# zzbuzzard/PATHS

Hardware: AMD Instinct MI355X
Metric: slides_per_sec_5level_K2048_D1024 (higher is better)
Workload: dtype f32 (products as 2 fp16 planes per operand = 22 bits, 3 fp16 MFMAs per block, fp32 accumulate); 1 GPU; 5-level PATHS recursion (forward, eval): K=2048 patches/level (level-0 grid 32x64, top_k 512, 10% background), D=1024 features, trans_dim 128 x 4 heads x 2 layers, LSTM ctx 256; 8 HBM-resident slides per GPU; slides_per_gpu=8, global_batch=8, levels=5, resident_batches_rotated=3, parallelism=slide-sharded x1 (no data-path collective)

## Files before the change

paths_amd/csrc/gemm_epi.h:

```cpp
#pragma once
#include "common.h"

namespace paths_epi {



struct TileView {
  char* base; int64_t ldb; uint32_t lane_off;
  __device__ TileView(const float* p, int64_t ld, int lane)
      : base(reinterpret_cast<char*>(const_cast<float*>(p))), ldb(ld * 4), lane_off((uint32_t)((4 * (lane >> 5)) * ld + (lane & 31)) * 4u) {}
  __device__ float* at(int trow, int tcol, int r) const {
    char* tile = base + (int64_t)trow * ldb + (int64_t)tcol * 4;
    const uint32_t off = lane_off + (uint32_t)((r & 3) + 8 * (r >> 2)) * (uint32_t)ldb;
    return reinterpret_cast<float*>(tile + off);
  }
  __device__ char* tile(int trow, int tcol) const { return base + (int64_t)trow * ldb + (int64_t)tcol * 4; }
  __device__ float* elem(char* tile_origin, int r) const {
    return reinterpret_cast<float*>(tile_origin + (lane_off + (uint32_t)((r & 3) + 8 * (r >> 2)) * (uint32_t)ldb));
  }
  __device__ float* at_clamped(int trow, int tcol, int r, int lane, int M) const {
    const int row = min(trow + c32_row(r, lane), M - 1);
    return reinterpret_cast<float*>(base + (int64_t)row * ldb + (int64_t)(tcol + (lane & 31)) * 4);
  }
};
// ... 220 lines not shown
      char* to = ovw.tile(trow, tcol); char* tx = xvw.tile(trow, tcol);
      if constexpr (RAW_O) {
        const f32x4* t4 = reinterpret_cast<const f32x4*>(o + ((int64_t)(trow >> 5) * (N >> 5) + (tcol >> 5)) * 1024) + lane;
#pragma unroll
        for (int q = 0; q < 4; ++q) {
          const f32x4 v = t4[64 * q];
          ov[s][4 * q] = v[0]; ov[s][4 * q + 1] = v[1]; ov[s][4 * q + 2] = v[2]; ov[s][4 * q + 3] = v[3];
        }
      }
      static_for<0, 16>([&](auto rc) __attribute__((always_inline)) {
        constexpr int r = decltype(rc)::value;
        if constexpr (FULL) {
          if constexpr (!RAW_O) ov[s][r] = *ovw.elem(to, r);
          if constexpr (WITH_Y) xv[s][r] = *xvw.elem(tx, r);
        } else {
          if constexpr (!RAW_O) ov[s][r] = *ovw.at_clamped(trow, tcol, r, lane, M);
          if constexpr (WITH_Y) xv[s][r] = *xvw.at_clamped(trow, tcol, r, lane, M);
        }
      });
    };
    static_for<0, (PD < NT ? PD : NT)>([&](auto tc) __attribute__((always_inline)) { load(tc); });
    static_for<0, NT>([&](auto tc) __attribute__((always_inline)) {
      constexpr int t = decltype(tc)::value, i = t % WTM, j = t / WTM, s = t % NB;
      if constexpr (t + PD < NT) load(std::integral_constant<int, t + PD>{});
      const int trow = row0 + 32 * i, tcol = col0 + 32 * j;
      if (tcol < N) {
        const float b = bias[tcol + (lane & 31)];
        char* th = hv.tile(trow, tcol); char* ty = yv.tile(trow, tcol); char* tt = tv.tile(trow, tcol);
        static_for<0, 16>([&](auto rc) __attribute__((always_inline)) {
          constexpr int r = decltype(rc)::value;
          const float tcv = tanh_acc(fmaf(acc[i][j][r], acc_scale, b));
          const float h = (RAW_O ? sigmoid_acc(ov[s][r]) : ov[s][r]) * tcv;
          if constexpr (FULL) {
            if constexpr (WITH_TC) *tv.elem(tt, r) = tcv;
            *hv.elem(th, r) = h;
            if constexpr (WITH_Y) *yv.elem(ty, r) = xv[s][r] + h;
          } else if (tile_row_ok<false>(trow, r, lane, M)) {
            if constexpr (WITH_TC) *tv.at_clamped(trow, tcol, r, lane, M) = tcv;
            *hv.at_clamped(trow, tcol, r, lane, M) = h;
            if constexpr (WITH_Y) *yv.at_clamped(trow, tcol, r, lane, M) = xv[s][r] + h;
          }
        });
      }
      __builtin_amdgcn_sched_barrier(0);
    });
  }
  template <int WTM, int WTN, int WGM, int WGN>
  __device__ __forceinline__ void run(f32x16 (&acc)[WTM][WTN], int row0, int col0, int lane, int, int, int M, float*) const {
    if (row0 + 32 * WTM <= M) run_impl<true>(acc, row0, col0, lane, M);
    else run_impl<false>(acc, row0, col0, lane, M);
  }
};

struct EpiBias {
  template <int WTM, int WTN>
  __device__ __forceinline__ void init(f32x16 (&acc)[WTM][WTN], int, int, int, int) const {
#pragma unroll
    for (int i = 0; i < WTM; ++i)
#pragma unroll
      for (int j = 0; j < WTN; ++j)
#pragma unroll
        for (int r = 0; r < 16; ++r) acc[i][j][r] = 0.f;
  }

  const float* bias; float* out; int64_t ldo; int N; int act;
  const float* residual; int64_t ldr; const float* mask; int64_t ldm; int accumulate;
  float acc_scale = 1.0f;
  template <bool FULL, int WTM, int WTN>
  __device__ __forceinline__ void run_impl(f32x16 (&acc)[WTM][WTN], int row0, int col0, int lane, int M) const {
    constexpr int NT = WTM * WTN;
    const TileView outv(out, ldo, lane), resv(residual, ldr, lane), maskv(mask, ldm, lane);
    float rv[2][16], mv[2][16], ov[2][16];
    const bool any_load = residual != nullptr || mask != nullptr || accumulate != 0;
    auto load = [&](auto tc) __attribute__((always_inline)) {
      constexpr int t = decltype(tc)::value, i = t % WTM, j = t / WTM, s = t & 1;
      const int trow = row0 + 32 * i, tcol = col0 + 32 * j;
      const int lcol = min(tcol + (lane & 31), N - 1) - (lane & 31);
#pragma unroll
      for (int r = 0; r < 16; ++r) {
        rv[s][r] = residual ? *tile_elem<FULL>(resv, trow, lcol, r, lane, M) : 0.f;
        mv[s][r] = mask ? *tile_elem<FULL>(maskv, trow, lcol, r, lane, M) : 1.f;
        ov[s][r] = accumulate ? *tile_elem<FULL>(outv, trow, lcol, r, lane, M) : 0.f;
      }
    };
    if (any_load) load(std::integral_constant<int, 0>{});
    static_for<0, NT>([&](auto tc) __attribute__((always_inline)) {
      constexpr int t = decltype(tc)::value, i = t % WTM, j = t / WTM, s = t & 1;
      if constexpr (t + 1 < NT) {
        if (any_load) load(std::integral_constant<int, t + 1>{});
      }
      const int trow = row0 + 32 * i, tcol = col0 + 32 * j;
      const int colr = tcol + (lane & 31);
      const float b = bias ? bias[min(colr, N - 1)] : 0.f;
      if (tcol < N) {
#pragma unroll
        for (int r = 0; r < 16; ++r) {
          float v = fmaf(acc[i][j][r], acc_scale, b);
          if (act == 1) v = fmaxf(v, 0.f);
          if (any_load) {
            if (!(mv[s][r] > 0.f)) v = 0.f;
            v += rv[s][r] + ov[s][r];
          }
          if (tile_row_ok<FULL>(trow, r, lane, M) && (tcol + 32 <= N || colr < N)) *tile_elem<FULL>(outv, trow, tcol, r, lane, M) = v;
        }
      }
      __builtin_amdgcn_sched_barrier(0);
// ... 188 lines not shown
```

paths_amd/csrc/gemm_x6.hip:

```cpp
#include "common.h"
#include "gemm_epi.h"
#include "finish_qkv.h"

#ifndef PATHS_X6_PART
#define PATHS_X6_PART 0
#endif

namespace {
using namespace paths_epi;

typedef __bf16 bf16x8 __attribute__((ext_vector_type(8)));
typedef _Float16 f16x8 __attribute__((ext_vector_type(8)));
typedef _Float16 f16x2 __attribute__((ext_vector_type(2)));
typedef __bf16 bf16x2 __attribute__((ext_vector_type(2)));
typedef float f32x2 __attribute__((ext_vector_type(2)));
typedef uint32_t u32x2 __attribute__((ext_vector_type(2)));
typedef uint32_t u32x4 __attribute__((ext_vector_type(4)));

__device__ __forceinline__ uint32_t pk_bf16(float a, float b) {
  f32x2 v = {a, b};
  return __builtin_bit_cast(uint32_t, __builtin_convertvector(v, bf16x2));
}
__device__ __forceinline__ float bf_lo(uint32_t p) { return __builtin_bit_cast(float, p << 16); }
__device__ __forceinline__ float bf_hi(uint32_t p) { return __builtin_bit_cast(float, p & 0xffff0000u); }

__device__ __forceinline__ uint32_t pk_f16(float a, float b) {
  f32x2 v = {a, b};
  return __builtin_bit_cast(uint32_t, __builtin_convertvector(v, f16x2));
}
__device__ __forceinline__ float h_lo(uint32_t p) { return (float)__builtin_bit_cast(f16x2, p)[0]; }
__device__ __forceinline__ float h_hi(uint32_t p) { return (float)__builtin_bit_cast(f16x2, p)[1]; }

constexpr int FRAG = 1024;
template <int NP> constexpr int planes_of() { return NP == 4 ? 2 : NP; }
template <int NP> constexpr int subt() { return planes_of<NP>() * FRAG; }

struct X6Operands {
  const float* A0; int64_t lda0; int K0;
  const int64_t* A0rows;
  const float* A1; int64_t lda1; int K1;
  const float* Aadd; int64_t ldadd;
  const char* Wt;
  int64_t w_group_stride;
  int M;
  const int64_t* num_ims;
  int rows_per_slide;
  float a_scale;
  int ksplit = 1;
};

template <int NP, int WTM, int WTN, int PF, bool ADD, bool ROWS, class Epi, int OCC = 1, bool A16 = false>
__global__ void __launch_bounds__(256) __attribute__((amdgpu_waves_per_eu(OCC, OCC)))
gemm_x6_kernel(X6Operands g, Epi epi) {
  static_assert(NP == 2 || NP == 3 || NP == 4, "two fp16 planes, three bf16 planes or two bf16 planes");
  static_assert(!A16 || (NP == 2 && ROWS), "fp16 A rows: two-plane fp16 split, row-pointer form");
  constexpr int PL = planes_of<NP>();
  constexpr bool A1P = A16 && !ADD;
  constexpr int PLA = A1P ? 1 : PL;
  constexpr int SUBT = subt<NP>();
  constexpr int SUBTA = PLA * FRAG;
  constexpr int NPROD = NP == 3 ? 6 : A1P ? 2 : 3;
  constexpr int BM = WTM * 64, BN = WTN * 64;
  constexpr int SA = 2 * WTM, SB = 2 * WTN;
  constexpr int STAGE = SA * SUBTA + SB * SUBT;
  constexpr int NA = BM / 64;
  constexpr int NPB = SB * PL, NB = (NPB + 3) / 4;
  static_assert(WTM % 2 == 0, "A fragment register slots alternate per accumulator row");
  extern __shared__ __attribute__((aligned(16))) char smem[];
  const int tid = threadIdx.x, lane = tid & 63, wave = __builtin_amdgcn_readfirstlane(tid >> 6), wm = wave >> 1, wn = wave & 1;

  const int nbx = gridDim.x, nby = gridDim.y, nblk = nbx * nby;
  int lin = blockIdx.y * nbx + blockIdx.x;
  {
    const int q = nblk >> 3, r = nblk & 7, xcd = lin & 7, j = lin >> 3;
    lin = (xcd < r ? xcd * (q + 1) : r * (q + 1) + (xcd - r) * q) + j;
  }
  constexpr int GM = 8;
  const int per_group = GM * nbx;
  const int grp = lin / per_group, in_grp = lin - grp * per_group;
  const int rows_in_grp = min(GM, nby - grp * GM);
  const int by = grp * GM + in_grp % rows_in_grp, bx = in_grp / rows_in_grp;
  const int m0 = by * BM, n0 = bx * BN;
  if (block_all_padding(g.num_ims, g.rows_per_slide, m0, BM, g.M)) return;

  const int arow = tid >> 2, ac = tid & 3;
  uint32_t aoff0[NA], aoff1[NA], aoffs[ADD ? NA : 1]; int awr[NA];
  typedef const f32x4 __attribute__((address_space(1))) * gptr_f4;
  typedef const u32x2 __attribute__((address_space(1))) * gptr_h4;
  gptr_f4 rowp[ROWS && !A16 ? NA : 1];
  gptr_h4 rowh[A16 ? NA : 1];
#pragma unroll
  for (int p = 0; p < NA; ++p) {
    const int row = p * 64 + arow;
    const int64_t grow = min(m0 + row, g.M - 1);
    aoff0[p] = ROWS ? 0u : (uint32_t)((grow * g.lda0 + 4 * ac) * 4);
    if constexpr (A16) rowh[p] = reinterpret_cast<gptr_h4>(static_cast<uintptr_t>(g.A0rows[grow]) + 8 * ac);
    else if constexpr (ROWS) rowp[p] = reinterpret_cast<gptr_f4>(static_cast<uintptr_t>(g.A0rows[grow]) + 16 * ac);
    aoff1[p] = (uint32_t)((grow * g.lda1 + 4 * ac) * 4);
    if constexpr (ADD) aoffs[p] = (uint32_t)((grow * g.ldadd + 4 * ac) * 4);
    awr[p] = (row >> 5) * SUBTA + (ac >> 1) * 512 + (row & 31) * 16 + (ac & 1) * 8;
  }
  const int K0w = g.ksplit > 1 ? g.K0 / g.ksplit : g.K0;
  const int kofs = g.ksplit > 1 ? (int)blockIdx.z * K0w : 0;
  if (kofs != 0) {
#pragma unroll
    for (int p = 0; p < NA; ++p) {
      aoff0[p] += (uint32_t)kofs * 4u;
      if constexpr (A16) rowh[p] += kofs >> 2;
      else if constexpr (ROWS) rowp[p] += kofs >> 2;
      if constexpr (ADD) aoffs[p] += (uint32_t)kofs * 4u;
    }
  }
  const int nk0 = K0w >> 4, nk = (K0w + g.K1) >> 4;
  const char* bbase[NB]; int bwr[NB];
#pragma unroll
  for (int i = 0; i < NB; ++i) {
    int pc = wave + 4 * i;
    if (pc >= NPB) pc -= 4;
    const int sub = pc / PL, pl = pc % PL;
    bbase[i] = g.Wt + ((int64_t)(n0 >> 5) + sub) * g.w_group_stride + pl * FRAG;
    bwr[i] = (A1P ? SA * SUBTA + sub * SUBT : (SA + sub) * SUBT) + pl * FRAG + lane * 16;
  }
  static_assert(PF == 1 || PF == 2, "one or two register sets");
  f32x4 sa[PF][NA], sadd[ADD ? PF : 1][ADD ? NA : 1]; u32x4 sbr[PF][NB];
  u32x2 sh[A16 ? PF : 1][A16 ? NA : 1];
  uint32_t hi[NA][2], mid[NP != 2 ? NA : 1][2], lo[NA][2];
  float* const anyA = const_cast<float*>(ROWS ? reinterpret_cast<const float*>(g.Wt) : g.A0);
  const auto rsA0 = __builtin_amdgcn_make_buffer_rsrc(anyA, 0, 0xFFFFFFFFu, 0x00020000);
  const auto rsA1 = __builtin_amdgcn_make_buffer_rsrc(g.A1 ? const_cast<float*>(g.A1) : anyA, 0, 0xFFFFFFFFu, 0x00020000);
  const auto rsAdd = __builtin_amdgcn_make_buffer_rsrc(ADD ? const_cast<float*>(g.Aadd) : anyA, 0, 0xFFFFFFFFu, 0x00020000);
  const auto rsW = __builtin_amdgcn_make_buffer_rsrc(const_cast<char*>(g.Wt), 0, 0xFFFFFFFFu, 0x00020000);
  const int lane16 = lane * 16;
  int bsoff[NB];
#pragma unroll
  for (int i = 0; i < NB; ++i) bsoff[i] = (int)(bbase[i] - g.Wt) + (kofs >> 4) * SUBT;
  auto gload_a = [&](int set, int q, int kt) {
// ... 34 lines not shown
        asm("v_pk_mul_f16 %0, %1, %2" : "=v"(hi[q][1]) : "v"(sh[set][q][1]), "v"(s2));
      }
      if (st == 1) *reinterpret_cast<u32x2*>(smem + buf * STAGE + awr[q]) = u32x2{hi[q][0], hi[q][1]};
    } else if constexpr (NP == 3) {
      if (st == 0) { hi[q][0] = pk_bf16(v[0], v[1]); hi[q][1] = pk_bf16(v[2], v[3]); }
      if (st == 1) { tf[q][0] = bf_lo(hi[q][0]); tf[q][1] = bf_hi(hi[q][0]); }
      if (st == 2) { v[0] -= tf[q][0]; v[1] -= tf[q][1]; }
      if (st == 3) { tf[q][0] = bf_lo(hi[q][1]); tf[q][1] = bf_hi(hi[q][1]); }
      if (st == 4) { v[2] -= tf[q][0]; v[3] -= tf[q][1]; }
      if (st == 5) { mid[q][0] = pk_bf16(v[0], v[1]); mid[q][1] = pk_bf16(v[2], v[3]); }
      if (st == 6) { tf[q][0] = bf_lo(mid[q][0]); tf[q][1] = bf_hi(mid[q][0]); }
      if (st == 7) { v[0] -= tf[q][0]; v[1] -= tf[q][1]; }
      if (st == 8) { tf[q][0] = bf_lo(mid[q][1]); tf[q][1] = bf_hi(mid[q][1]); }
      if (st == 9) { v[2] -= tf[q][0]; v[3] -= tf[q][1]; }
      if (st == 10) { lo[q][0] = pk_bf16(v[0], v[1]); lo[q][1] = pk_bf16(v[2], v[3]); }
      if (st == 11) {
        char* d = smem + buf * STAGE + awr[q];
        *reinterpret_cast<u32x2*>(d) = u32x2{hi[q][0], hi[q][1]};
        *reinterpret_cast<u32x2*>(d + FRAG) = u32x2{mid[q][0], mid[q][1]};
        *reinterpret_cast<u32x2*>(d + 2 * FRAG) = u32x2{lo[q][0], lo[q][1]};
      }
    } else if constexpr (NP == 4) {
      if (st == 0) { hi[q][0] = pk_bf16(v[0], v[1]); hi[q][1] = pk_bf16(v[2], v[3]); }
      if (st == 1) { tf[q][0] = bf_lo(hi[q][0]); tf[q][1] = bf_hi(hi[q][0]); }
      if (st == 2) { v[0] -= tf[q][0]; v[1] -= tf[q][1]; }
      if (st == 3) { tf[q][0] = bf_lo(hi[q][1]); tf[q][1] = bf_hi(hi[q][1]); }
      if (st == 4) { v[2] -= tf[q][0]; v[3] -= tf[q][1]; }
      if (st == 5) { mid[q][0] = pk_bf16(v[0], v[1]); mid[q][1] = pk_bf16(v[2], v[3]); }
      if (st == 6) {
        char* d = smem + buf * STAGE + awr[q];
        *reinterpret_cast<u32x2*>(d) = u32x2{hi[q][0], hi[q][1]};
        *reinterpret_cast<u32x2*>(d + FRAG) = u32x2{mid[q][0], mid[q][1]};
      }
    } else {
      if (st == 0) v *= g.a_scale;
      if (st == 1) { hi[q][0] = pk_f16(v[0], v[1]); hi[q][1] = pk_f16(v[2], v[3]); }
      if (st == 2) {
        asm("v_fma_mixlo_f16 %0, %1, -1.0, %2 op_sel_hi:[1,0,0]" : "=v"(lo[q][0]) : "v"(hi[q][0]), "v"(v[0]));
        asm("v_fma_mixlo_f16 %0, %1, -1.0, %2 op_sel_hi:[1,0,0]" : "=v"(lo[q][1]) : "v"(hi[q][1]), "v"(v[2]));
      }
      if (st == 3) {
        asm("v_fma_mixhi_f16 %0, %1, -1.0, %2 op_sel:[1,0,0] op_sel_hi:[1,0,0]" : "+v"(lo[q][0]) : "v"(hi[q][0]), "v"(v[1]));
        asm("v_fma_mixhi_f16 %0, %1, -1.0, %2 op_sel:[1,0,0] op_sel_hi:[1,0,0]" : "+v"(lo[q][1]) : "v"(hi[q][1]), "v"(v[3]));
      }
      if (st == 4) {
        char* d = smem + buf * STAGE + awr[q];
        *reinterpret_cast<u32x2*>(d) = u32x2{hi[q][0], hi[q][1]};
        *reinterpret_cast<u32x2*>(d + FRAG) = u32x2{lo[q][0], lo[q][1]};
      }
    }
  };
  auto swrite_b = [&](int set, int q, int buf) { *reinterpret_cast<u32x4*>(smem + buf * STAGE + bwr[q]) = sbr[set][q]; };

  f32x16 acc[WTM][WTN];
  epi.template init<WTM, WTN>(acc, m0 + wm * WTM * 32, n0 + wn * WTN * 32, lane, g.M);

  const char* sA = smem + (wm * WTM) * SUBTA + lane * 16;
  const char* sB = A1P ? smem + SA * SUBTA + (wn * WTN) * SUBT + lane * 16 : smem + (SA + wn * WTN) * SUBT + lane * 16;
  u32x4 fa[2][PLA], fb[2][WTN][PL];
  auto read_a = [&](int buf, int i, int slot, int p) { fa[slot][p] = *reinterpret_cast<const u32x4*>(sA + buf * STAGE + i * SUBTA + p * FRAG); };
  auto read_b = [&](int buf, int j, int slot, int p) { fb[slot][j][p] = *reinterpret_cast<const u32x4*>(sB + buf * STAGE + j * SUBT + p * FRAG); };
  constexpr int RG = WTN * NPROD;
  auto one_mfma = [&](int gq, int sb) __attribute__((always_inline)) {
    const int i = gq / RG, j = (gq % RG) / NPROD, t = gq % NPROD, sl = i & 1;
    if constexpr (NP == 3) {
      constexpr int PA_[6] = {2, 0, 1, 1, 0, 0}, PB_[6] = {0, 2, 1, 0, 1, 0};
      acc[i][j] = __builtin_amdgcn_mfma_f32_32x32x16_bf16(__builtin_bit_cast(bf16x8, fa[sl][PA_[t]]), __builtin_bit_cast(bf16x8, fb[sb][j][PB_[t]]), acc[i][j], 0, 0, 0);
    } else if constexpr (NP == 4) {
      constexpr int PA_[3] = {1, 0, 0}, PB_[3] = {0, 1, 0};
      acc[i][j] = __builtin_amdgcn_mfma_f32_32x32x16_bf16(__builtin_bit_cast(bf16x8, fa[sl][PA_[t]]), __builtin_bit_cast(bf16x8, fb[sb][j][PB_[t]]), acc[i][j], 0, 0, 0);
    } else if constexpr (A1P) {
      constexpr int PB_[2] = {1, 0};
      acc[i][j] = __builtin_amdgcn_mfma_f32_32x32x16_f16(__builtin_bit_cast(f16x8, fa[sl][0]), __builtin_bit_cast(f16x8, fb[sb][j][PB_[t]]), acc[i][j], 0, 0, 0);
    } else {
      constexpr int PA_[3] = {1, 0, 0}, PB_[3] = {0, 1, 0};
      acc[i][j] = __builtin_amdgcn_mfma_f32_32x32x16_f16(__builtin_bit_cast(f16x8, fa[sl][PA_[t]]), __builtin_bit_cast(f16x8, fb[sb][j][PB_[t]]), acc[i][j], 0, 0, 0);
    }
  };
  constexpr int AG = (WTM - 1) * RG;
  constexpr auto fits = [](int spg) constexpr {
    return PF == 1 ? ((NS + spg - 1) / spg) * NA + NB <= AG : (NS * NA + spg - 1) / spg + NB <= AG;
  };
  constexpr int SPG = fits(1) ? 1 : fits(2) ? 2 : fits(3) ? 3 : 4;
  static_assert(fits(SPG), "staging does not fit before the barrier");
  constexpr int GPC = (NS + SPG - 1) / SPG;
  constexpr int GA2 = (NS * NA + SPG - 1) / SPG;
  constexpr int TS = PF == 1 ? GPC * NA + NB : GA2 + NB + NA + NB;
  static_assert(TS <= WTM * RG, "staging does not fit in a stage");
  constexpr int AR0 = RG / 2;
  auto staging_slot = [&](auto sc, int kt, auto bufc, auto m1c, auto m2c) __attribute__((always_inline)) {
    constexpr int s = decltype(sc)::value, buf = decltype(bufc)::value;
    constexpr bool more1 = decltype(m1c)::value, more2 = decltype(m2c)::value;
    constexpr int set = PF == 2 ? (buf ^ 1) : 0;
    if constexpr (PF == 1) {
      if constexpr (s < GPC * NA) {
        constexpr int q = s / GPC, g0 = s % GPC;
        if constexpr (more1) {
          static_for<g0 * SPG, (g0 + 1) * SPG < NS ? (g0 + 1) * SPG : NS>([&](auto mc) __attribute__((always_inline)) {
            a_step(set, q, decltype(mc)::value, buf ^ 1);
          });
        }
        if constexpr (more2 && g0 == GPC - 1) gload_a(set, q, kt + 1 + PF);
      } else if constexpr (s < TS) {
        if constexpr (more1) swrite_b(set, s - GPC * NA, buf ^ 1);
        if constexpr (more2) gload_b(set, s - GPC * NA, kt + 1 + PF);
      }
    } else {
      if constexpr (s < GA2) {
// ... 29 lines not shown
      constexpr int gq = decltype(gc)::value, gr = gq % RG;
      one_mfma(gq, sb);
      if constexpr (more1) {
        static_for<2 * gr, 2 * gr + 2>([&](auto fc) __attribute__((always_inline)) {
          constexpr int f = decltype(fc)::value;
          if constexpr (f < PLA) read_a(buf ^ 1, 0, 0, f);
          else if constexpr (f < PLA + PL * WTN) read_b(buf ^ 1, (f - PLA) / PL, sb ^ 1, (f - PLA) % PL);
        });
      }
      staging_slot(std::integral_constant<int, gq>{}, kt, bufc, m1c, m2c);
      __builtin_amdgcn_sched_barrier(0);
    });
  };
  constexpr std::integral_constant<int, 0> I0{};
  constexpr std::integral_constant<int, 1> I1{};
  constexpr std::true_type T{};
  constexpr std::false_type F{};

#pragma unroll
  for (int q = 0; q < NA; ++q) gload_a(0, q, 0);
#pragma unroll
  for (int q = 0; q < NB; ++q) gload_b(0, q, 0);
#pragma unroll
  for (int q = 0; q < NA; ++q)
#pragma unroll
    for (int st = 0; st < NS; ++st) a_step(0, q, st, 0);
#pragma unroll
  for (int q = 0; q < NB; ++q) swrite_b(0, q, 0);
#pragma unroll
  for (int sidx = 1; sidx <= PF; ++sidx) {
#pragma unroll
    for (int q = 0; q < NA; ++q) gload_a(PF == 2 ? (sidx & 1) : 0, q, sidx);
#pragma unroll
    for (int q = 0; q < NB; ++q) gload_b(PF == 2 ? (sidx & 1) : 0, q, sidx);
  }
  __syncthreads();
#pragma unroll
  for (int p = 0; p < PLA; ++p) read_a(0, 0, 0, p);
#pragma unroll
  for (int j = 0; j < WTN; ++j)
#pragma unroll
    for (int p = 0; p < PL; ++p) read_b(0, j, 0, p);
  for (int kt = 0; kt < nk - 2 * PF; kt += 2) {
    __builtin_amdgcn_sched_barrier(0);
    stage_body(kt, I0, T, T);
    stage_body(kt + 1, I1, T, T);
  }
  if constexpr (PF == 2) {
    stage_body(nk - 4, I0, T, T);
    stage_body(nk - 3, I1, T, F);
  }
  stage_body(nk - 2, I0, T, F);
  stage_body(nk - 1, I1, F, F);
  __syncthreads();
  epi.template run<WTM, WTN, 2, 2>(acc, m0 + wm * WTM * 32, n0 + wn * WTN * 32, lane, wm, wn, g.M, reinterpret_cast<float*>(smem));
}

template <int NP>
__global__ void x6_pack_kernel(const float* __restrict__ w, int64_t ldw, uint16_t* __restrict__ out, int N, int Npad, int K, float wscale) {
  const int64_t i = blockIdx.x * (int64_t)blockDim.x + threadIdx.x;
  if (i >= (int64_t)Npad * K) return;
  const int n = (int)(i / K), k = (int)(i % K);
  const float v = n < N ? w[(int64_t)n * ldw + k] * wscale : 0.f;
  uint16_t* o = out + ((int64_t)(n >> 5) * (K >> 4) + (k >> 4)) * (subt<NP>() / 2) + ((k >> 3) & 1) * 256 + (n & 31) * 8 + (k & 7);
  if constexpr (NP == 3) {
    const __bf16 h = (__bf16)v; const float r1 = v - (float)h;
    const __bf16 m = (__bf16)r1; const float r2 = r1 - (float)m;
    const __bf16 l = (__bf16)r2;
    o[0] = __builtin_bit_cast(uint16_t, h); o[FRAG / 2] = __builtin_bit_cast(uint16_t, m); o[FRAG] = __builtin_bit_cast(uint16_t, l);
  } else if constexpr (NP == 4) {
    const __bf16 h = (__bf16)v; const float r1 = v - (float)h;
    const __bf16 m = (__bf16)r1;
    o[0] = __builtin_bit_cast(uint16_t, h); o[FRAG / 2] = __builtin_bit_cast(uint16_t, m);
  } else {
    const _Float16 h = (_Float16)v; const float r1 = v - (float)h;
    const _Float16 l = (_Float16)r1;
    o[0] = __builtin_bit_cast(uint16_t, h); o[FRAG / 2] = __builtin_bit_cast(uint16_t, l);
  }
}

template <int NP>
__global__ void x6_pack_t_kernel(const float* __restrict__ w, int64_t ldw, uint16_t* __restrict__ out, int N, int Npad, int K, int Kvalid) {
  static_assert(NP == 3 || NP == 4, "bf16 planes (scale 1)");
  const int64_t i = blockIdx.x * (int64_t)blockDim.x + threadIdx.x;
  if (i >= (int64_t)Npad * (K >> 3)) return;
  const int n = (int)(i % Npad), k0 = (int)(i / Npad) * 8;
  uint16_t h[8], m[8], l[8];
#pragma unroll
  for (int j = 0; j < 8; ++j) {
    const int k = k0 + j;
    const float v = (n < N && k < Kvalid) ? w[(int64_t)k * ldw + n] : 0.f;
    const __bf16 hh = (__bf16)v; const float r1 = v - (float)hh;
    const __bf16 mm = (__bf16)r1; const float r2 = r1 - (float)mm;
    const __bf16 ll = (__bf16)r2;
    h[j] = __builtin_bit_cast(uint16_t, hh); m[j] = __builtin_bit_cast(uint16_t, mm); l[j] = __builtin_bit_cast(uint16_t, ll);
  }
  uint16_t* o = out + ((int64_t)(n >> 5) * (K >> 4) + (k0 >> 4)) * (subt<NP>() / 2) + ((k0 >> 3) & 1) * 256 + (n & 31) * 8;
  typedef uint16_t u16x8 __attribute__((ext_vector_type(8)));
  *reinterpret_cast<u16x8*>(o) = u16x8{h[0], h[1], h[2], h[3], h[4], h[5], h[6], h[7]};
  *reinterpret_cast<u16x8*>(o + FRAG / 2) = u16x8{m[0], m[1], m[2], m[3], m[4], m[5], m[6], m[7]};
  if constexpr (NP == 3) *reinterpret_cast<u16x8*>(o + FRAG) = u16x8{l[0], l[1], l[2], l[3], l[4], l[5], l[6], l[7]};
}

template <int NP, int WTM, int WTN, int PF, bool ADD, bool ROWS, class Epi, int OCC = 1, bool A16 = false>
int launch_x6_np(const X6Operands& g, int Npad, const Epi& epi, hipStream_t stream, const char* name) {
  constexpr int BM = WTM * 64, BN = WTN * 64;
  constexpr size_t lds = 2ull * (2 * WTM * ((A16 && !ADD) ? FRAG : subt<NP>()) + 2 * WTN * subt<NP>());
  const int K = g.K0 + g.K1;
// ... 77 lines not shown
  if (planes == 2) return launch_x6_np<2, WTM, WTN, PF, ADD, false>(g, Npad, epi, stream, name);
  return paths_set_error(PATHS_EINVAL, "%s: planes must be 3 (bf16 x6) or 2 (fp16 x3), got %d", name, planes);
}

constexpr int H_OCC = 3;
constexpr int H_TRAIN_OCC = 2;

inline int plane_count(int planes) { return planes == 4 ? 2 : planes; }
inline int64_t group_stride(int planes, int Kpacked) { return (int64_t)(Kpacked / 16) * plane_count(planes) * FRAG; }
inline bool pow2(float x) { int e; return x > 0.f && frexpf(x, &e) == 0.5f; }
inline bool h16_scale_ok(float a_scale) { return pow2(a_scale) && a_scale >= 1.0f && a_scale <= 32768.0f; }

}

extern "C" {

#if PATHS_X6_PART == 0 || PATHS_X6_PART == 1
int64_t paths_x6_packed_bytes(int Npad, int K, int planes) { return (int64_t)Npad * K * 2 * plane_count(planes); }

int paths_x6_pack_weights(const float* w, int64_t ldw, void* out, int N, int Npad, int K, int planes, float w_scale, hipStream_t stream) {
  PATHS_REQUIRE(N > 0 && Npad >= N && Npad % 32 == 0 && K % 16 == 0, "x6_pack_weights: bad shape N=%d Npad=%d K=%d", N, Npad, K);
  PATHS_REQUIRE((uintptr_t)out % 16 == 0, "x6_pack_weights: out must be 16-byte aligned");
  PATHS_REQUIRE(((planes == 3 || planes == 4) && w_scale == 1.0f) || (planes == 2 && pow2(w_scale)), "x6_pack_weights: planes 3 / 4 (bf16) with w_scale 1, or planes 2 with a power-of-two w_scale");
  const int64_t n = (int64_t)Npad * K;
  const dim3 grid((unsigned)((n + 255) / 256));
  if (planes == 4) hipLaunchKernelGGL(x6_pack_kernel<4>, grid, dim3(256), 0, stream, w, ldw, reinterpret_cast<uint16_t*>(out), N, Npad, K, 1.0f);
  else if (planes == 3) hipLaunchKernelGGL(x6_pack_kernel<3>, grid, dim3(256), 0, stream, w, ldw, reinterpret_cast<uint16_t*>(out), N, Npad, K, 1.0f);
  else hipLaunchKernelGGL(x6_pack_kernel<2>, grid, dim3(256), 0, stream, w, ldw, reinterpret_cast<uint16_t*>(out), N, Npad, K, w_scale);
  PATHS_LAUNCH_CHECK("x6_pack_weights");
  return PATHS_OK;
}

int paths_x6_pack_weights_t(const float* w, int64_t ldw, void* out, int N, int Npad, int K, int Kvalid, int planes, hipStream_t stream) {
  PATHS_REQUIRE(N > 0 && Npad >= N && Npad % 32 == 0 && K % 16 == 0 && Kvalid > 0 && Kvalid <= K, "x6_pack_weights_t: bad shape N=%d Npad=%d K=%d Kvalid=%d", N, Npad, K, Kvalid);
  PATHS_REQUIRE(w != nullptr && out != nullptr && (uintptr_t)out % 16 == 0, "x6_pack_weights_t: null / unaligned operand");
  PATHS_REQUIRE(planes == 3 || planes == 4, "x6_pack_weights_t: planes 3 or 4 (bf16)");
  const int64_t n = (int64_t)Npad * (K / 8);
  const dim3 grid((unsigned)((n + 255) / 256));
  if (planes == 4) hipLaunchKernelGGL(x6_pack_t_kernel<4>, grid, dim3(256), 0, stream, w, ldw, reinterpret_cast<uint16_t*>(out), N, Npad, K, Kvalid);
  else hipLaunchKernelGGL(x6_pack_t_kernel<3>, grid, dim3(256), 0, stream, w, ldw, reinterpret_cast<uint16_t*>(out), N, Npad, K, Kvalid);
  PATHS_LAUNCH_CHECK("x6_pack_weights_t");
  return PATHS_OK;
}

}
namespace {
template <bool A16>
int lstm_cell_x6(const float* x, int64_t ldx, const int64_t* x_rows, const float* h0, int64_t ldh0, const float* c0, int64_t ldc0,
                 const void* w_gates_x6, const float* b_gates, const void* w_mem_x6, const float* b_mem,
                 float* state_out, int64_t ldso, float* y, int64_t ldy, float* ws_o, float* save_frm, float* save_tc,
                 const float* hp, const int* hp_row, int M, int D, int Hc, const int64_t* num_ims, int rows_per_slide,
                 int phases, int planes, float wg_scale, float wm_scale, float a_scale, hipStream_t stream) {
  PATHS_REQUIRE(D % 256 == 0 && Hc % 64 == 0, "lstm_cell_x6: D (%d) must be a multiple of 256 and Hc (%d) of 64", D, Hc);
  if constexpr (A16) {
    PATHS_REQUIRE(x_rows != nullptr && x == nullptr && planes == 2, "lstm_cell_x6_h16: fp16 rows are given as x_rows (planes = 2)");
    PATHS_REQUIRE(h16_scale_ok(a_scale), "lstm_cell_x6_h16: a_scale must be a power of two in [1, 2^15]");
  }
  PATHS_REQUIRE(hp != nullptr || (h0 == nullptr) == (c0 == nullptr), "lstm_cell_x6: h0 and c0 must both be given or both be null");
  PATHS_REQUIRE((hp == nullptr) == (hp_row == nullptr) && (hp == nullptr || h0 == nullptr),
                "lstm_cell_x6: hp/hp_row come together and replace h0 (the h half of the gate GEMM was done per parent)");
  PATHS_REQUIRE(planes == 3 || (pow2(wg_scale) && pow2(wm_scale) && pow2(a_scale)), "lstm_cell_x6: scales must be powers of two");
  PATHS_REQUIRE(x_rows == nullptr || (h0 == nullptr && y == nullptr && save_tc == nullptr), "lstm_cell_x6: x_rows (rows addressed in place) excludes h0, y and the training saves");
  if (planes == 3) wg_scale = wm_scale = a_scale = 1.0f;
  const char* wg = reinterpret_cast<const char*>(w_gates_x6);
  const int64_t gs = group_stride(planes, 2 * D);
  const float sg = 1.0f / (wg_scale * a_scale), sm = 1.0f / (wm_scale * a_scale);
  X6Operands g{x, ldx, D, x_rows, h0, h0 ? ldh0 : 0, h0 ? D : 0, nullptr, 0, wg, gs, M, num_ims, rows_per_slide, a_scale};
  const bool small_m = planes == 2 && M <= 8192 && (h0 == nullptr);
  if (phases & 1) {
    EpiLstmC e{b_gates, c0, ldc0, state_out + D, ldso, save_frm, (int64_t)3 * Hc, hp, (int64_t)3 * Hc + D, hp_row, sg};
    int rc;
    if constexpr (A16) {
      rc = small_m ? launch_x6_np<2, 2, 3, 2, false, true, decltype(e), 1, true>(g, 3 * Hc, e, stream, "lstm_cell_x6_h16(c, 128-row tiles)")
                   : launch_x6_np<2, 4, 3, 1, false, true, decltype(e), 1, true>(g, 3 * Hc, e, stream, "lstm_cell_x6_h16(c)");
    } else if (small_m) rc = x_rows ? launch_x6_np<2, 2, 3, 2, false, true>(g, 3 * Hc, e, stream, "lstm_cell_x6(c, 128-row tiles)")
                             : launch_x6_np<2, 2, 3, 2, false, false>(g, 3 * Hc, e, stream, "lstm_cell_x6(c, 128-row tiles)");
    else rc = launch_x6<4, 3, 1, false>(planes, g, 3 * Hc, e, stream, "lstm_cell_x6(c)");
    if (rc) return rc;
  }
  const bool o_raw = y == nullptr && save_tc == nullptr && save_frm == nullptr;
  if (phases & 2) {
    X6Operands go = g;
    go.Wt = wg + (int64_t)(3 * Hc / 32) * gs;
    int rc;
    if (o_raw) {
      EpiLstmORaw e{b_gates + 3 * Hc, ws_o, D, D, hp, (int64_t)3 * Hc + D, hp_row, 3 * Hc, sg};
      if constexpr (A16) {
        rc = small_m ? launch_x6_np<2, 2, 4, 2, false, true, decltype(e), 1, true>(go, D, e, stream, "lstm_cell_x6_h16(o, raw, 128-row tiles)")
                     : launch_x6_np<2, 4, 4, 1, false, true, decltype(e), 1, true>(go, D, e, stream, "lstm_cell_x6_h16(o, raw)");
      } else if (small_m) rc = x_rows ? launch_x6_np<2, 2, 4, 2, false, true>(go, D, e, stream, "lstm_cell_x6(o, raw, 128-row tiles)")
                               : launch_x6_np<2, 2, 4, 2, false, false>(go, D, e, stream, "lstm_cell_x6(o, raw, 128-row tiles)");
      else rc = launch_x6<4, 4, 1, false>(planes, go, D, e, stream, "lstm_cell_x6(o, raw)");
    } else {
      EpiLstmO e{b_gates + 3 * Hc, ws_o, D, D, hp, (int64_t)3 * Hc + D, hp_row, 3 * Hc, sg};
      if constexpr (A16) rc = launch_x6_np<2, 4, 4, 1, false, true, decltype(e), 1, true>(go, D, e, stream, "lstm_cell_x6_h16(o)");
      else rc = launch_x6<4, 4, 1, false>(planes, go, D, e, stream, "lstm_cell_x6(o)");
    }
    if (rc) return rc;
  }
  if (phases & 4) {
    X6Operands gh{state_out + D, ldso, Hc, nullptr, nullptr, 0, 0, nullptr, 0, reinterpret_cast<const char*>(w_mem_x6), group_stride(planes, Hc), M, num_ims, rows_per_slide, a_scale};
    int rc;
    PATHS_REQUIRE(save_tc == nullptr || y != nullptr, "lstm_cell_x6: save_tc (training) needs y");
    PATHS_REQUIRE(planes == 2 || planes == 3, "lstm_cell_x6: planes must be 3 (bf16 x6) or 2 (fp16 x3), got %d", planes);
    if (save_tc != nullptr) {
      EpiLstmH<true, true> e{b_mem, ws_o, D, x, ldx, state_out, ldso, y, ldy, D, save_tc, sm};
      if (planes == 2) rc = launch_x6_np<2, 2, 2, 2, false, false, decltype(e), H_TRAIN_OCC>(gh, D, e, stream, "lstm_cell_x6(h, save, 128x128)");
      else rc = launch_x6_np<3, 4, 4, 1, false, false>(gh, D, e, stream, "lstm_cell_x6(h, save)");
    } else if (y != nullptr) {
      EpiLstmH<true, false> e{b_mem, ws_o, D, x, ldx, state_out, ldso, y, ldy, D, nullptr, sm};
      rc = launch_x6<4, 4, 1, false>(planes, gh, D, e, stream, "lstm_cell_x6(h)");
    } else if (o_raw) {
      EpiLstmH<false, false, true> e{b_mem, ws_o, D, x, ldx, state_out, ldso, nullptr, 0, D, nullptr, sm};
      if (planes == 2) rc = launch_x6_np<2, 2, 2, 2, false, false, decltype(e), H_OCC>(gh, D, e, stream, "lstm_cell_x6(h, raw o, 128x128)");
      else rc = launch_x6_np<3, 4, 4, 1, false, false>(gh, D, e, stream, "lstm_cell_x6(h, raw o)");
    } else {
      EpiLstmH<false, false> e{b_mem, ws_o, D, x, ldx, state_out, ldso, nullptr, 0, D, nullptr, sm};
      if (planes == 2) rc = launch_x6_np<2, 2, 2, 2, false, false, decltype(e), H_OCC>(gh, D, e, stream, "lstm_cell_x6(h, no y, 128x128)");
      else rc = launch_x6_np<3, 4, 4, 1, false, false>(gh, D, e, stream, "lstm_cell_x6(h, no y)");
    }
    if (rc) return rc;
  }
  return PATHS_OK;
}
}
extern "C" {

int paths_lstm_cell_x6(const float* x, int64_t ldx, const int64_t* x_rows, const float* h0, int64_t ldh0, const float* c0, int64_t ldc0,
                       const void* w_gates_x6, const float* b_gates, const void* w_mem_x6, const float* b_mem,
                       float* state_out, int64_t ldso, float* y, int64_t ldy, float* ws_o, float* save_frm, float* save_tc,
                       const float* hp, const int* hp_row, int M, int D, int Hc, const int64_t* num_ims, int rows_per_slide,
                       int phases, int planes, float wg_scale, float wm_scale, float a_scale, hipStream_t stream) {
  return lstm_cell_x6<false>(x, ldx, x_rows, h0, ldh0, c0, ldc0, w_gates_x6, b_gates, w_mem_x6, b_mem, state_out, ldso, y, ldy, ws_o, save_frm,
                             save_tc, hp, hp_row, M, D, Hc, num_ims, rows_per_slide, phases, planes, wg_scale, wm_scale, a_scale, stream);
}

int paths_lstm_cell_x6_h16(const float* x, int64_t ldx, const int64_t* x_rows, const float* h0, int64_t ldh0, const float* c0, int64_t ldc0,
                           const void* w_gates_x6, const float* b_gates, const void* w_mem_x6, const float* b_mem,
                           float* state_out, int64_t ldso, float* y, int64_t ldy, float* ws_o, float* save_frm, float* save_tc,
                           const float* hp, const int* hp_row, int M, int D, int Hc, const int64_t* num_ims, int rows_per_slide,
                           int phases, int planes, float wg_scale, float wm_scale, float a_scale, hipStream_t stream) {
  return lstm_cell_x6<true>(x, ldx, x_rows, h0, ldh0, c0, ldc0, w_gates_x6, b_gates, w_mem_x6, b_mem, state_out, ldso, y, ldy, ws_o, save_frm,
                            save_tc, hp, hp_row, M, D, Hc, num_ims, rows_per_slide, phases, planes, wg_scale, wm_scale, a_scale, stream);
}

#endif
#if PATHS_X6_PART == 0 || PATHS_X6_PART == 2
int64_t paths_importance_proj_x6_workspace(int M) { return 2ll * ((M + 127) / 128 * 4) * 8 * 1024 * 4; }

}
namespace {
// ... 222 lines not shown
```

paths_amd/ops.py:

```python
from __future__ import annotations

import math
import os
from typing import Dict, List, Optional

import torch

from . import _lib

LOG2E = 1.4426950408889634
QKV_IMAGES = os.environ.get("PATHS_QKV_IMAGES", "1") != "0"
TAIL_WS = os.environ.get("PATHS_TAIL_WS", "1") != "0"
TLAYER_WS = os.environ.get("PATHS_TLAYER_WS", "1") != "0"
SPLITK_IMPORTANCE = os.environ.get("PATHS_SPLITK_IMPORTANCE", "1") != "0"
FUSE_QKV = int(os.environ.get("PATHS_FUSE_QKV", "2"))
KERNEL_TIMER = None
TIMER_ALL = False


def timed(name: str, fn, meta=None, detail: bool = True):
    if KERNEL_TIMER is None or (detail and not TIMER_ALL):
        return fn()
    return KERNEL_TIMER(name, fn, meta or {})
GEMM_MODE = os.environ.get("PATHS_GEMM_MODE", "h3")
# ... 773 lines not shown
                    _lib.call("paths_importance_qkv_x6" + h16, *args, 3, 0, st)
                    fused["finish"] = lambda: _lib.call("paths_importance_qkv_x6", *args, 4, 1, _lib.stream())
                else:
                    _lib.call("paths_importance_qkv_x6" + h16, *args, 5, 0, st)
                fused["qkv_img"], fused["ws"] = qkv_img, ws
                return
            splitk_ws = None
            if splitk:
                splitk_ws = torch.empty((int(_lib.load().paths_importance_proj_x6_workspace(M)),), device=dev, dtype=torch.uint8)
            _lib.call("paths_importance_proj_x6" + (h16 if src is None else ""), p(src), D, p(x_rows) if src is None else None, p(add),
                      add.stride(1) if add is not None else 0,
                      p(wip), *common[:-1], split_planes(), wip_s, a_scale(), p(splitk_ws), common[-1])
        else:
            assert add is None
            _lib.call("paths_importance_proj", p(src), D, p(lvl_pack["w_ip_fwd"]), *common)

    if importance_out is not None:
        assert importance_out.shape == (B, N) and importance_out.is_contiguous() and importance_out.dtype == torch.float32
        importance = importance_out
    else:
        importance = torch.zeros((B, N), **f32) if skip_padding else torch.empty((B, N), **f32)
    if mc.lstm:
        Hc = lstm_pack["Hc"]
        Dp = D + Hc
        state_out = torch.empty((B, N, Dp), **f32)
        y = None if (x6 and (not generic or generic_add)) else torch.empty((B, N, D), **f32)
        ws_o = torch.empty(((M + 255) // 256 * 256, D), **f32)
        hp, hp_row = None, None
        if parent is not None:
            assert state_prev is None
            c0t = parent["c0"]
            assert c0t.shape == (B, N, Hc) and c0t.is_contiguous()
            ld, h0, c0 = Hc, None, c0t.data_ptr()
            hp, hp_row = p(parent["hp"]), p(parent["hp_row"])
        elif state_prev is not None:
            assert state_prev.shape[:2] == (B, N) and state_prev.shape[2] == Dp and state_prev.stride(2) == 1
            assert state_prev.stride(0) == N * state_prev.stride(1), "state rows must be uniformly strided"
            ld = state_prev.stride(1)
            h0, c0 = state_prev.data_ptr(), state_prev.data_ptr() + 4 * D
        else:
            ld, h0, c0 = 0, None, None

        def lstm(phases):
            if x6:
                (wg, wg_s), (wm, wm_s) = _x6_of(lstm_pack, "w_gates"), _x6_of(lstm_pack, "w_mem")
                _lib.call("paths_lstm_cell_x6" + h16, p(fts), D, p(x_rows), h0, ld, c0, ld, p(wg), p(lstm_pack["b_gates"]), p(wm), p(lstm_pack["b_mem"]),
                          p(state_out), Dp, p(y), D, p(ws_o), None, None, hp, hp_row, M, D, Hc, nim, N, phases,
                          split_planes(), wg_s, wm_s, a_scale(), st)
            else:
                _lib.call("paths_lstm_cell", p(fts), D, h0, ld, c0, ld, p(lstm_pack["w_gates"]), p(lstm_pack["b_gates"]),
                          p(lstm_pack["w_mem"]), p(lstm_pack["b_mem"]), p(state_out), Dp, p(y), D,
                          p(ws_o), None, None, hp, hp_row, M, D, Hc, nim, N, phases, st)

        if KERNEL_TIMER is None:
            lstm(7)
        else:
            timed("lstm_gate_c", lambda: lstm(1))
            timed("lstm_gate_o", lambda: lstm(2), {"rows": N, "B": B, "K": D if h0 is None else 2 * D, "Ncols": D, "parent_partials": parent is not None,
                                                   "x6": x6, "planes": split_planes() if x6 else 0}, detail=False)
            timed("lstm_mem_to_out", lambda: lstm(4))
        if generic_add:
            timed("importance_proj", lambda: importance_proj_generic_add(mc, lvl_pack, fts, x_rows, state_out, locs, num_ims, B, N, D,
                                                                         1 if mc.importance_mode == "mul" else 0, importance, tokens, skip_padding, pe_tab=pe_tab,
                                                                         x_rows_h16=x_rows_h16))
        elif x6 and not generic:
            timed("importance_proj", lambda: importance_proj(fts, 1 if mc.importance_mode == "mul" else 0, importance, add=state_out))
        else:
            timed("importance_proj", lambda: importance_proj(y, 1 if mc.importance_mode == "mul" else 0, importance))
        del ws_o
    else:
        importance_proj(fts, 0, importance)
        hctx = None
        if state_prev is not None and mc.hierarchical_ctx:
            assert state_prev.shape == (B, N, D) and state_prev.stride(2) == 1 and state_prev.stride(0) == N * state_prev.stride(1)
            Hh = lvl_pack["wh1"].shape[0]
            assert Hh % 128 == 0, "hierarchical_ctx_mlp_hidden_dim must be a multiple of 128 for lstm=false"
            hid = torch.empty((B, N, Hh), **f32)
            hctx = torch.empty((B, N, D), **f32)
            _lib.call("paths_linear_f32", p(state_prev), state_prev.stride(1), p(lvl_pack["wh1"]), p(lvl_pack["bh1"]), p(hid), Hh,
                      M, Hh, Hh, D, 1, st)
            _lib.call("paths_linear_f32", p(hid), Hh, p(lvl_pack["wh2"]), p(lvl_pack["bh2"]), p(hctx), D, M, D, D, Hh, 0, st)
        state_out = torch.empty((B, N, D), **f32)
        _lib.call("paths_scale_add_rows", p(fts), p(importance), p(hctx) if hctx is not None else None, p(num_ims), N, D, M,
                  1 if mc.importance_mode == "mul" else 0, p(state_out), st)
        scratch_imp = torch.empty((B, N), **f32)
        importance_proj(state_out, 0, scratch_imp)

    out = {"ctx_patch": state_out, "importance": importance, "tokens": tokens, "num_ims": num_ims}
    if "qkv_img" in fused:
        out["qkv_img"], out["qkv_finish"], out["_qkv_ws"] = fused["qkv_img"], fused.get("finish"), fused["ws"]
    return out


def parent_partials(lstm_pack, state_out: torch.Tensor, keep_idx: torch.Tensor, keep_count: torch.Tensor,
                    kept_rows: Optional[torch.Tensor] = None) -> torch.Tensor:
    B, N, Dp = state_out.shape
    Hc = lstm_pack["Hc"]
    D = Dp - Hc
    G = 3 * Hc + D
    cap = keep_idx.shape[1]
    f32 = dict(device=state_out.device, dtype=torch.float32)
    st = _lib.stream()
    p = _lib.ptr
    hp = torch.empty((B * cap, G), **f32)
    if kept_rows is not None:
        assert use_x6(D, Hc) and G % 256 == 0 and split_planes() == 2 and kept_rows.shape == (B, cap) and kept_rows.dtype == torch.int64
        wg, wg_s = _x6_of(lstm_pack, "w_gates")
        timed("parent_gemm", lambda: _lib.call("paths_gemm_rows_nt_x6", p(kept_rows), p(wg), 2 * D, D, p(hp), G, B * cap, G, D, 2, wg_s, a_scale(), st))
        return hp
    hk = torch.empty((B * cap, D), **f32)
    _lib.call("paths_gather_kept_rows", p(state_out), N, Dp, p(keep_idx), cap, p(keep_count), D, B, p(hk), st)
    if use_x6(D, Hc) and G % 256 == 0:
        wg, wg_s = _x6_of(lstm_pack, "w_gates")
# ... 260 lines not shown
```

Before: 3761 slides/s.

## Fuse LSTM mem_to_out GEMM and output gate into one kernel launch

After: 3672 slides/s, median of 2. -2.4%, worse.

```diff
diff --git a/paths_amd/csrc/gemm_epi.h b/paths_amd/csrc/gemm_epi.h
--- a/paths_amd/csrc/gemm_epi.h
+++ b/paths_amd/csrc/gemm_epi.h
@@ -296,6 +296,81 @@
   }
 };
 
+struct EpiLstmOH {
+  EpiLstmORaw g;
+  const float* bias_m; float sm;
+  float* h1; int64_t ldh;
+  const int64_t* num_ims; int rows_per_slide;
+  uint32_t scratch_bytes, h1_bytes;
+  typedef uint32_t u32x4 __attribute__((ext_vector_type(4)));
+  template <int WTM, int WTN>
+  __device__ __forceinline__ void zero(f32x16 (&acc)[WTM][WTN]) const {
+#pragma unroll
+    for (int i = 0; i < WTM; ++i)
+#pragma unroll
+      for (int j = 0; j < WTN; ++j)
+#pragma unroll
+        for (int r = 0; r < 16; ++r) acc[i][j][r] = 0.f;
+  }
+  __device__ __forceinline__ int slot(int trow, int tcol) const { return ((trow >> 5) * (g.N >> 5) + (tcol >> 5)) * 4096; }
+  template <int WTM, int WTN>
+  __device__ __forceinline__ void park(f32x16 (&acc)[WTM][WTN], int row0, int col0, int lane) const {
+    const auto rs = __builtin_amdgcn_make_buffer_rsrc(g.o, 0, scratch_bytes, 0x00020000);
+    static_for<0, WTM * WTN>([&](auto tc) __attribute__((always_inline)) {
+      constexpr int t = decltype(tc)::value, i = t % WTM, j = t / WTM;
+      const int tcol = col0 + 32 * j;
+      const float b = bias_m[tcol + (lane & 31)];
+      const int so = slot(row0 + 32 * i, tcol);
+#pragma unroll
+      for (int q = 0; q < 4; ++q) {
+        const f32x4 v = f32x4{tanh_acc(fmaf(acc[i][j][4 * q], sm, b)), tanh_acc(fmaf(acc[i][j][4 * q + 1], sm, b)),
+                              tanh_acc(fmaf(acc[i][j][4 * q + 2], sm, b)), tanh_acc(fmaf(acc[i][j][4 * q + 3], sm, b))};
+        __builtin_amdgcn_raw_buffer_store_b128(__builtin_bit_cast(u32x4, v), rs, lane * 16, so + 1024 * q, 0);
+      }
+      __builtin_amdgcn_sched_barrier(0);
+    });
+  }
+  template <int WTM, int WTN>
+  __device__ __forceinline__ void init(f32x16 (&acc)[WTM][WTN], int row0, int col0, int lane, int M) const {
+    g.template init<WTM, WTN>(acc, row0, col0, lane, M);
+  }
+  template <int WTM, int WTN>
+  __device__ __forceinline__ void run(f32x16 (&acc)[WTM][WTN], int row0, int col0, int lane, int M) const {
+    static_assert(WTM == 4, "one wave = one 128-row block of the mem_to_out launch");
+    if (row0 >= M || block_all_padding(num_ims, rows_per_slide, row0, 32 * WTM, M)) return;
+    constexpr int NT = WTM * WTN, PD = NT >= 4 ? 3 : 1, NB = PD + 1;
+    const auto rs = __builtin_amdgcn_make_buffer_rsrc(g.o, 0, scratch_bytes, 0x00020000);
+    const auto rh = __builtin_amdgcn_make_buffer_rsrc(h1, 0, h1_bytes, 0x00020000);
+    const auto rb = __builtin_amdgcn_make_buffer_rsrc(const_cast<float*>(g.bias), 0, (uint32_t)g.N * 4u, 0x00020000);
+    const uint32_t ldb = (uint32_t)ldh * 4u;
+    const uint32_t lane_off = (uint32_t)(4 * (lane >> 5)) * ldb + (uint32_t)(lane & 31) * 4u;
+    float tv[NB][16];
+    auto load = [&](auto tc) __attribute__((always_inline)) {
+      constexpr int t = decltype(tc)::value, i = t % WTM, j = t / WTM, s = t % NB;
+      const int so = slot(row0 + 32 * i, col0 + 32 * j);
+#pragma unroll
+      for (int q = 0; q < 4; ++q) {
+        const f32x4 v = __builtin_bit_cast(f32x4, __builtin_amdgcn_raw_buffer_load_b128(rs, lane * 16, so + 1024 * q, 0));
+        tv[s][4 * q] = v[0]; tv[s][4 * q + 1] = v[1]; tv[s][4 * q + 2] = v[2]; tv[s][4 * q + 3] = v[3];
+      }
+    };
+    static_for<0, (PD < NT ? PD : NT)>([&](auto tc) __attribute__((always_inline)) { load(tc); });
+    static_for<0, NT>([&](auto tc) __attribute__((always_inline)) {
+      constexpr int t = decltype(tc)::value, i = t % WTM, j = t / WTM, s = t % NB;
+      if constexpr (t + PD < NT) load(std::integral_constant<int, t + PD>{});
+      const int trow = row0 + 32 * i, tcol = col0 + 32 * j;
+      const float b = __builtin_bit_cast(float, __builtin_amdgcn_raw_buffer_load_b32(rb, (lane & 31) * 4, tcol * 4, 0));
+      const uint32_t origin = (uint32_t)trow * ldb + (uint32_t)tcol * 4u;
+      static_for<0, 16>([&](auto rc) __attribute__((always_inline)) {
+        constexpr int r = decltype(rc)::value;
+        const float h = sigmoid_acc(fmaf(acc[i][j][r], g.acc_scale, b)) * tv[s][r];
+        __builtin_amdgcn_raw_buffer_store_b32(__builtin_bit_cast(uint32_t, h), rh, (int)(lane_off + (origin + (uint32_t)((r & 3) + 8 * (r >> 2)) * ldb)), 0, 0);
+      });
+      __builtin_amdgcn_sched_barrier(0);
+    });
+  }
+};
+
 struct EpiBias {
   template <int WTM, int WTN>
   __device__ __forceinline__ void init(f32x16 (&acc)[WTM][WTN], int, int, int, int) const {
diff --git a/paths_amd/csrc/gemm_x6.hip b/paths_amd/csrc/gemm_x6.hip
--- a/paths_amd/csrc/gemm_x6.hip
+++ b/paths_amd/csrc/gemm_x6.hip
@@ -49,9 +49,24 @@
   int ksplit = 1;
 };
 
-template <int NP, int WTM, int WTN, int PF, bool ADD, bool ROWS, class Epi, int OCC = 1, bool A16 = false>
-__global__ void __launch_bounds__(256) __attribute__((amdgpu_waves_per_eu(OCC, OCC)))
-gemm_x6_kernel(X6Operands g, Epi epi) {
+template <int BM, int BN>
+__device__ __forceinline__ void x6_tile_origin(int& m0, int& n0) {
+  const int nbx = gridDim.x, nby = gridDim.y, nblk = nbx * nby;
+  int lin = blockIdx.y * nbx + blockIdx.x;
+  {
+    const int q = nblk >> 3, r = nblk & 7, xcd = lin & 7, j = lin >> 3;
+    lin = (xcd < r ? xcd * (q + 1) : r * (q + 1) + (xcd - r) * q) + j;
+  }
+  constexpr int GM = 8;
+  const int per_group = GM * nbx;
+  const int grp = lin / per_group, in_grp = lin - grp * per_group;
+  const int rows_in_grp = min(GM, nby - grp * GM);
+  const int by = grp * GM + in_grp % rows_in_grp, bx = in_grp / rows_in_grp;
+  m0 = by * BM; n0 = bx * BN;
+}
+
+template <int NP, int WTM, int WTN, int PF, bool ADD, bool ROWS, bool A16, class Seed>
+__device__ __forceinline__ void x6_mainloop(const X6Operands& g, f32x16 (&acc)[WTM][WTN], char* smem, const int m0, const int n0, Seed&& seed) {
   static_assert(NP == 2 || NP == 3 || NP == 4, "two fp16 planes, three bf16 planes or two bf16 planes");
   static_assert(!A16 || (NP == 2 && ROWS), "fp16 A rows: two-plane fp16 split, row-pointer form");
   constexpr int PL = planes_of<NP>();
@@ -66,22 +81,7 @@
   constexpr int NA = BM / 64;
   constexpr int NPB = SB * PL, NB = (NPB + 3) / 4;
   static_assert(WTM % 2 == 0, "A fragment register slots alternate per accumulator row");
-  extern __shared__ __attribute__((aligned(16))) char smem[];
   const int tid = threadIdx.x, lane = tid & 63, wave = __builtin_amdgcn_readfirstlane(tid >> 6), wm = wave >> 1, wn = wave & 1;
-
-  const int nbx = gridDim.x, nby = gridDim.y, nblk = nbx * nby;
-  int lin = blockIdx.y * nbx + blockIdx.x;
-  {
-    const int q = nblk >> 3, r = nblk & 7, xcd = lin & 7, j = lin >> 3;
-    lin = (xcd < r ? xcd * (q + 1) : r * (q + 1) + (xcd - r) * q) + j;
-  }
-  constexpr int GM = 8;
-  const int per_group = GM * nbx;
-  const int grp = lin / per_group, in_grp = lin - grp * per_group;
-  const int rows_in_grp = min(GM, nby - grp * GM);
-  const int by = grp * GM + in_grp % rows_in_grp, bx = in_grp / rows_in_grp;
-  const int m0 = by * BM, n0 = bx * BN;
-  if (block_all_padding(g.num_ims, g.rows_per_slide, m0, BM, g.M)) return;
 
   const int arow = tid >> 2, ac = tid & 3;
   uint32_t aoff0[NA], aoff1[NA], aoffs[ADD ? NA : 1]; int awr[NA];
@@ -222,8 +222,7 @@
   };
   auto swrite_b = [&](int set, int q, int buf) { *reinterpret_cast<u32x4*>(smem + buf * STAGE + bwr[q]) = sbr[set][q]; };
 
-  f32x16 acc[WTM][WTN];
-  epi.template init<WTM, WTN>(acc, m0 + wm * WTM * 32, n0 + wn * WTN * 32, lane, g.M);
+  seed();
 
   const char* sA = smem + (wm * WTM) * SUBTA + lane * 16;
   const char* sB = A1P ? smem + SA * SUBTA + (wn * WTN) * SUBT + lane * 16 : smem + (SA + wn * WTN) * SUBT + lane * 16;
@@ -359,8 +358,43 @@
   }
   stage_body(nk - 2, I0, T, F);
   stage_body(nk - 1, I1, F, F);
+}
+
+template <int NP, int WTM, int WTN, int PF, bool ADD, bool ROWS, class Epi, int OCC = 1, bool A16 = false>
+__global__ void __launch_bounds__(256) __attribute__((amdgpu_waves_per_eu(OCC, OCC)))
+gemm_x6_kernel(X6Operands g, Epi epi) {
+  extern __shared__ __attribute__((aligned(16))) char smem[];
+  const int tid = threadIdx.x, lane = tid & 63, wave = __builtin_amdgcn_readfirstlane(tid >> 6), wm = wave >> 1, wn = wave & 1;
+  int m0, n0;
+  x6_tile_origin<WTM * 64, WTN * 64>(m0, n0);
+  if (block_all_padding(g.num_ims, g.rows_per_slide, m0, WTM * 64, g.M)) return;
+  f32x16 acc[WTM][WTN];
+  x6_mainloop<NP, WTM, WTN, PF, ADD, ROWS, A16>(g, acc, smem, m0, n0, [&]() __attribute__((always_inline)) {
+    epi.template init<WTM, WTN>(acc, m0 + wm * WTM * 32, n0 + wn * WTN * 32, lane, g.M);
+  });
   __syncthreads();
   epi.template run<WTM, WTN, 2, 2>(acc, m0 + wm * WTM * 32, n0 + wn * WTN * 32, lane, wm, wn, g.M, reinterpret_cast<float*>(smem));
+}
+
+template <int WTM, int WTN, bool A16, class Epi>
+__global__ void __launch_bounds__(256) __attribute__((amdgpu_waves_per_eu(1, 1)))
+lstm_oh_x6_kernel(X6Operands gb, X6Operands ga, Epi epi) {
+  extern __shared__ __attribute__((aligned(16))) char smem[];
+  const int tid = threadIdx.x, lane = tid & 63, wave = __builtin_amdgcn_readfirstlane(tid >> 6), wm = wave >> 1, wn = wave & 1;
+  int m0, n0;
+  x6_tile_origin<WTM * 64, WTN * 64>(m0, n0);
+  if (block_all_padding(ga.num_ims, ga.rows_per_slide, m0, WTM * 64, ga.M)) return;
+  const int row0 = m0 + wm * WTM * 32, col0 = n0 + wn * WTN * 32;
+  f32x16 acc[WTM][WTN];
+  x6_mainloop<2, WTM, WTN, 1, false, false, false>(gb, acc, smem, m0, n0, [&]() __attribute__((always_inline)) {
+    epi.template zero<WTM, WTN>(acc);
+  });
+  epi.template park<WTM, WTN>(acc, row0, col0, lane);
+  __syncthreads();
+  x6_mainloop<2, WTM, WTN, 1, false, true, A16>(ga, acc, smem, m0, n0, [&]() __attribute__((always_inline)) {
+    epi.template init<WTM, WTN>(acc, row0, col0, lane, ga.M);
+  });
+  epi.template run<WTM, WTN>(acc, row0, col0, (int)__builtin_amdgcn_mbcnt_hi(~0u, __builtin_amdgcn_mbcnt_lo(~0u, 0u)), ga.M);
 }
 
 template <int NP>
@@ -544,6 +578,8 @@
                  const float* hp, const int* hp_row, int M, int D, int Hc, const int64_t* num_ims, int rows_per_slide,
                  int phases, int planes, float wg_scale, float wm_scale, float a_scale, hipStream_t stream) {
   PATHS_REQUIRE(D % 256 == 0 && Hc % 64 == 0, "lstm_cell_x6: D (%d) must be a multiple of 256 and Hc (%d) of 64", D, Hc);
+  PATHS_REQUIRE(phases > 0 && (phases & ~15) == 0 && !((phases & 8) && (phases & 6)),
+                "lstm_cell_x6: phases (%d) is a mask of 1 (c), 2 (o gate), 4 (mem_to_out), 8 (o gate + mem_to_out in one launch, excludes 2 and 4)", phases);
   if constexpr (A16) {
     PATHS_REQUIRE(x_rows != nullptr && x == nullptr && planes == 2, "lstm_cell_x6_h16: fp16 rows are given as x_rows (planes = 2)");
     PATHS_REQUIRE(h16_scale_ok(a_scale), "lstm_cell_x6_h16: a_scale must be a power of two in [1, 2^15]");
@@ -589,6 +625,24 @@
       else rc = launch_x6<4, 4, 1, false>(planes, go, D, e, stream, "lstm_cell_x6(o)");
     }
     if (rc) return rc;
+  }
+  if (phases & 8) {
+    PATHS_REQUIRE(o_raw && !small_m && planes == 2 && x_rows != nullptr && ws_o != nullptr,
+                  "lstm_cell_x6: phase 8 (fused o gate + mem_to_out) is the inference form (no y, no saves) on row pointers, planes = 2, M > 8192");
+    PATHS_REQUIRE(Hc % 32 == 0 && Hc >= 128 && ldso % 4 == 0 && (uintptr_t)(state_out + D) % 16 == 0 && (uintptr_t)w_mem_x6 % 16 == 0 && (uintptr_t)wg % 16 == 0,
+                  "lstm_cell_x6: phase 8 needs Hc %% 32 == 0, Hc >= 128 and 16-byte aligned operands");
+    PATHS_REQUIRE((int64_t)M * ldso * 4 < (int64_t)1 << 32 && (int64_t)((M + 255) / 256 * 256) * D * 4 < (int64_t)1 << 32, "lstm_cell_x6: state_out or the gate scratch larger than 4 GiB");
+    X6Operands go = g;
+    go.Wt = wg + (int64_t)(3 * Hc / 32) * gs;
+    X6Operands gh{state_out + D, ldso, Hc, nullptr, nullptr, 0, 0, nullptr, 0, reinterpret_cast<const char*>(w_mem_x6), group_stride(planes, Hc), M, num_ims, rows_per_slide, a_scale};
+    EpiLstmOH e{EpiLstmORaw{b_gates + 3 * Hc, ws_o, D, D, hp, (int64_t)3 * Hc + D, hp_row, 3 * Hc, sg}, b_mem, sm, state_out, ldso, num_ims, rows_per_slide,
+                (uint32_t)((int64_t)((M + 255) / 256 * 256) * D * 4), (uint32_t)((int64_t)M * ldso * 4)};
+    auto kern = lstm_oh_x6_kernel<4, 4, A16, EpiLstmOH>;
+    constexpr size_t lds = 2ull * (8 + 8) * subt<2>();
+    const char* name = A16 ? "lstm_cell_x6_h16(o + h fused)" : "lstm_cell_x6(o + h fused)";
+    PATHS_LDS_OPT_IN(kern, lds, name);
+    hipLaunchKernelGGL(kern, dim3(D / 256, (M + 255) / 256, 1), dim3(256), lds, stream, gh, go, e);
+    PATHS_LAUNCH_CHECK(name);
   }
   if (phases & 4) {
     X6Operands gh{state_out + D, ldso, Hc, nullptr, nullptr, 0, 0, nullptr, 0, reinterpret_cast<const char*>(w_mem_x6), group_stride(planes, Hc), M, num_ims, rows_per_slide, a_scale};
diff --git a/paths_amd/ops.py b/paths_amd/ops.py
--- a/paths_amd/ops.py
+++ b/paths_amd/ops.py
@@ -849,13 +849,22 @@
                           p(lstm_pack["w_mem"]), p(lstm_pack["b_mem"]), p(state_out), Dp, p(y), D,
                           p(ws_o), None, None, hp, hp_row, M, D, Hc, nim, N, phases, st)
 
+        fuse_oh = x6 and split_planes() == 2 and x_rows is not None and y is None and M > 8192
         if KERNEL_TIMER is None:
-            lstm(7)
+            if fuse_oh:
+                lstm(1)
+                lstm(8)
+            else:
+                lstm(7)
         else:
             timed("lstm_gate_c", lambda: lstm(1))
-            timed("lstm_gate_o", lambda: lstm(2), {"rows": N, "B": B, "K": D if h0 is None else 2 * D, "Ncols": D, "parent_partials": parent is not None,
-                                                   "x6": x6, "planes": split_planes() if x6 else 0}, detail=False)
-            timed("lstm_mem_to_out", lambda: lstm(4))
+            meta = {"rows": N, "B": B, "K": D if h0 is None else 2 * D, "Ncols": D, "parent_partials": parent is not None,
+                    "x6": x6, "planes": split_planes() if x6 else 0}
+            if fuse_oh:
+                timed("lstm_gate_o", lambda: lstm(8), dict(meta, K=D + Hc, fused_mem_to_out=True), detail=False)
+            else:
+                timed("lstm_gate_o", lambda: lstm(2), meta, detail=False)
+                timed("lstm_mem_to_out", lambda: lstm(4))
         if generic_add:
             timed("importance_proj", lambda: importance_proj_generic_add(mc, lvl_pack, fts, x_rows, state_out, locs, num_ims, B, N, D,
                                                                          1 if mc.importance_mode == "mul" else 0, importance, tokens, skip_padding, pe_tab=pe_tab,
```
